# homenc/HElib

Hardware: NVIDIA H100
Metric: ctxt_mults_per_s (higher is better)
Workload: dtype u64

## Files before the change

### helib_b200/csrc/hb_device_v1.cuh

```cuda
#pragma once
#include <utility>
#include "hb_device.cuh"

#define HB1_RS 17
#define HB1_BS 273

__device__ __forceinline__ void hb_group_sync(int group, int nthreads) {
#ifdef HB_SIM
  cusim::bar_sync(1 + group, nthreads);
#else
  asm volatile("bar.sync %0, %1;" ::"r"(1 + group), "r"(nthreads) : "memory");
#endif
}

__device__ __forceinline__ void hb1_mac128(u64& hi, u64& lo, u64 a, u64 b) {
#ifdef HB_SIM
  hb_mac128(hi, lo, a, b);
#else
  asm("{\n\t.reg .u64 pl, ph;\n\t"
      "mul.lo.u64 pl, %2, %3;\n\t"
      "mul.hi.u64 ph, %2, %3;\n\t"
      "add.cc.u64 %0, %0, pl;\n\t"
      "addc.u64 %1, %1, ph;\n\t}"
      : "+l"(lo), "+l"(hi)
      : "l"(a), "l"(b));
#endif
}


__device__ __forceinline__ u64 hb1_mulwide(unsigned a, unsigned b) {
#ifdef HB_SIM
  return (u64)a * b;
#else
  u64 r; asm("mul.wide.u32 %0, %1, %2;" : "=l"(r) : "r"(a), "r"(b)); return r;
#endif
}
__device__ __forceinline__ u64 hb1_mulhi_approx(u64 a, u64 b) {
  const unsigned alo = (unsigned)a, ahi = (unsigned)(a >> 32), blo = (unsigned)b, bhi = (unsigned)(b >> 32);
  return hb1_mulwide(ahi, bhi) + (u64)__umulhi(alo, bhi) + (u64)__umulhi(ahi, blo);
}
struct Hb1Mod {
  u64 nq, qb, qb2;
  unsigned qt, qsh;
};
#define HB1_MOD(M, P) Hb1Mod M; M.nq = (P).nq; M.qb = (P).qb; M.qb2 = (P).qb + (P).qb; M.qt = (P).qt; M.qsh = (P).qsh
template <bool SP>
__device__ __forceinline__ u64 hb1_shoup4(u64 y, u64 w, u64 ws, const Hb1Mod& M) {
  const u64 hi = hb1_mulhi_approx(y, ws);
  if (SP) {
    const unsigned tl = (unsigned)hi * M.qt;
    const unsigned ylo = (unsigned)y, yhi = (unsigned)(y >> 32), wlo = (unsigned)w, whi = (unsigned)(w >> 32);
    const u64 R = hb1_mulwide(ylo, wlo) - hi;
    const unsigned rhi = (unsigned)(R >> 32) + yhi * wlo + ylo * whi - (tl << M.qsh);
    return ((u64)rhi << 32) | (unsigned)R;
  }
  return y * w + hi * M.nq;
}
__device__ __forceinline__ u64 hb1_csub(u64 x, u64 m) {
  const u64 d = x - m;
  return (i64)d < 0 ? x : d;
}
__device__ __forceinline__ u64 hb1_csub_hi(u64 x, u64 m) {
#ifdef HB_SIM
  if ((unsigned)(x >> 32) > (unsigned)(m >> 32)) x -= m;
  return x;
#else
  unsigned xl = (unsigned)x, xh = (unsigned)(x >> 32);
  asm("{ .reg .pred p; setp.gt.u32 p, %1, %3; @p sub.cc.u32 %0, %0, %2; @p subc.u32 %1, %1, %3; }"
      : "+r"(xl), "+r"(xh) : "r"((unsigned)m), "r"((unsigned)(m >> 32)));
  return ((u64)xh << 32) | xl;
#endif
}
template <bool SP>
__device__ __forceinline__ void hb1_ct(u64& x, u64& y, u64 w, u64 ws, const Hb1Mod& M) {
  const u64 xr = hb1_csub_hi(x, M.qb);
  const u64 t = hb1_shoup4<SP>(y, w, ws, M);
  x = xr + t;
  y = xr - t + M.qb;
}
template <bool SP>
__device__ __forceinline__ void hb1_gs(u64& x, u64& y, u64 w, u64 ws, const Hb1Mod& M) {
  const u64 s = x + y;
  const u64 d = x - y + M.qb2;
  x = hb1_csub_hi(s, M.qb);
  y = hb1_shoup4<SP>(d, w, ws, M);
}
__device__ __forceinline__ u64 hb1_canon4(u64 x, u64 q) {
  x = hb1_csub(x, q + q);
  return hb1_csub(x, q);
}
__device__ __forceinline__ u64 hb1_canon_fwd(u64 x, u64 q, u64 qb) {
  x = hb1_csub_hi(x, qb);
  x = hb1_csub(x, q + q);
  x = hb1_csub(x, q);
  return hb1_csub(x, q);
}
__device__ __forceinline__ u64 hb1_canon_inv(u64 x, u64 q) {
  x = hb1_csub(x, q + q);
  x = hb1_csub(x, q);
  return hb1_csub(x, q);
}

template <int I> struct HbC {
  static constexpr int value = I;
  __device__ constexpr operator int() const { return I; }
};
template <class F, int... I>
__device__ __forceinline__ void hb1_unroll_seq(F&& f, std::integer_sequence<int, I...>) { (f(HbC<I>{}), ...); }
template <int N, class F>
__device__ __forceinline__ void hb1_unroll(F&& f) { hb1_unroll_seq(f, std::make_integer_sequence<int, N>{}); }

struct Hb1TwReg {
  ulonglong2 t[15];
  template <int K, int G> __device__ __forceinline__ ulonglong2 get() const { return t[(1 << K) - 1 + G]; }
  template <class F> __device__ __forceinline__ void load(F&& f) {
    hb1_unroll<4>([&](auto k) { hb1_unroll<(1 << k)>([&](auto g) { t[(1 << k) - 1 + g] = f((int)k, (int)g); }); });
  }
};
struct Hb1TwPtr {
  const ulonglong2* p[4];
  template <int K, int G> __device__ __forceinline__ ulonglong2 get() const { return p[K][G]; }
};
template <bool SP, class TW>
__device__ __forceinline__ void hb1_r16_fwd(u64 (&a)[16], const TW& tw, const Hb1Mod& M) {
  hb1_unroll<4>([&](auto k) {
    constexpr int d = 8 >> k;
    hb1_unroll<(1 << k)>([&](auto g) {
      const ulonglong2 w = tw.template get<k, g>();
      hb1_unroll<d>([&](auto o) { hb1_ct<SP>(a[g * 2 * d + o], a[g * 2 * d + o + d], w.x, w.y, M); });
    });
  });
}
template <bool SP, class TW>
__device__ __forceinline__ void hb1_r16_inv(u64 (&a)[16], const TW& tw, const Hb1Mod& M) {
  hb1_unroll<4>([&](auto kr) {
    constexpr int k = 3 - kr, d = 8 >> k;
    hb1_unroll<(1 << k)>([&](auto g) {
      const ulonglong2 w = tw.template get<k, g>();
      hb1_unroll<d>([&](auto o) { hb1_gs<SP>(a[g * 2 * d + o], a[g * 2 * d + o + d], w.x, w.y, M); });
    });
  });
}
__device__ __forceinline__ unsigned hb1_brev4(unsigned x) {
  return ((x & 1u) << 3) | ((x & 2u) << 1) | ((x & 4u) >> 1) | ((x & 8u) >> 3);
}

struct Hb1BlkJob {
  int logN, epi, lazy;
  HbRows rows;
  u64 scal[HB_MAXROWS], scal_s[HB_MAXROWS];
  int nitems;
  const u64* src[HB_MAXB];
  u64* dst[HB_MAXB];
  u64* dst2[HB_MAXB];
};

__device__ __forceinline__ void hb1_cp8(u64* dst_smem, const u64* src) {
#ifdef HB_SIM
  *dst_smem = *src;
#else
  unsigned sa = (unsigned)__cvta_generic_to_shared(dst_smem);
  asm volatile("cp.async.ca.shared.global [%0], [%1], 8;" ::"r"(sa), "l"(src) : "memory");
#endif
}
__device__ __forceinline__ void hb1_cp_commit() {
#ifndef HB_SIM
  asm volatile("cp.async.commit_group;" ::: "memory");
#endif
}
template <int N> __device__ __forceinline__ void hb1_cp_wait() {
#ifndef HB_SIM
  asm volatile("cp.async.wait_group %0;" ::"n"(N) : "memory");
#endif
}

__device__ __forceinline__ void hb1_bulk_store128(u64* gdst, const u64* ssrc) {
#ifdef HB_SIM
  for (int i = 0; i < 16; i++) gdst[i] = ssrc[i];
#else
  asm volatile("cp.async.bulk.global.shared::cta.bulk_group [%0], [%1], 128;"
               ::"l"(gdst), "r"((unsigned)__cvta_generic_to_shared(ssrc)) : "memory");
  asm volatile("cp.async.bulk.commit_group;" ::: "memory");
#endif
}
__device__ __forceinline__ void hb1_fence_async() {
#ifndef HB_SIM
  asm volatile("fence.proxy.async.shared::cta;" ::: "memory");
#endif
}
__device__ __forceinline__ void hb1_bulk_wait_read() {
#ifndef HB_SIM
  asm volatile("cp.async.bulk.wait_group.read 0;" ::: "memory");
#endif
}
__device__ __forceinline__ void hb1_bulk_wait_all() {
#ifndef HB_SIM
  asm volatile("cp.async.bulk.wait_group 0;" ::: "memory");
#endif
}

#define HB1_STAGE (16 * HB1_BS + 8)

struct Hb1Unit { int rowi, ug, it; };
__device__ __forceinline__ Hb1Unit hb1_unit_next(Hb1Unit x, int G, int nitems) {
  if (++x.it == nitems) { x.it = 0; if (++x.ug == G) { x.ug = 0; ++x.rowi; } }
  return x;
}
__device__ __forceinline__ Hb1Unit hb1_unit(long u, int G, int nitems) {
  Hb1Unit x;
  const unsigned per_row = (unsigned)(G * nitems), uu = (unsigned)u;
  x.rowi = (int)(uu / per_row);
  const int rem = (int)(uu - (unsigned)x.rowi * per_row);
  x.ug = rem / nitems;
  x.it = rem - x.ug * nitems;
  return x;
}
__device__ __forceinline__ bool hb1_units(const Hb1BlkJob& J, int G, long& ubeg, long& uend) {
  const long U = (long)J.rows.n * G * J.nitems;
  ubeg = U * blockIdx.x / gridDim.x; uend = U * (blockIdx.x + 1) / gridDim.x;
  return ubeg < uend;
}
__device__ __forceinline__ Hb1TwPtr hb1_tw1(const ulonglong2* TW1, int tid) {
  Hb1TwPtr tw1;
  tw1.p[0] = TW1 + (tid >> 4) * 16; tw1.p[1] = tw1.p[0] + 1; tw1.p[2] = tw1.p[0] + 3; tw1.p[3] = tw1.p[0] + 7;
  return tw1;
}
__device__ __forceinline__ unsigned hb1_blk_reload(const HbPrimeDev& P, const ulonglong2* tw, int n1, int ug, int tid, Hb1Mod& M,
                                                   ulonglong2* TW1, Hb1TwReg& tw2) {
  const int blk1 = tid >> 4, lo = tid & 15, hi = tid >> 4, blk2 = tid & 15;
  M.nq = P.nq; M.qb = P.qb; M.qb2 = P.qb + P.qb; M.qt = P.qt; M.qsh = P.qsh;
  const unsigned b1 = hb_brev((ug << 4) + blk1, n1), b2 = hb_brev((ug << 4) + blk2, n1);
  if (lo < 15) {
    int e = lo, k = e >= 7 ? 3 : (e >= 3 ? 2 : (e >= 1 ? 1 : 0));
    int g = e - ((1 << k) - 1);
    TW1[blk1 * 16 + e] = tw[((size_t)1 << (n1 + k)) + ((size_t)b1 << k) + g];
  }
  tw2.load([&](int k, int g) { return tw[((size_t)1 << (n1 + 4 + k)) + ((size_t)b2 << (4 + k)) + ((size_t)hi << k) + g]; });
  __syncthreads();
  return b1;
}

template <bool SP>
__global__ void __launch_bounds__(256, 2) k1_fwd_blk(const HbPrimeDev* __restrict__ primes, const HB_GRID_CONSTANT Hb1BlkJob J) {
  HB_SMEM_DECL
  u64* S = HB_SMEM;
  u64* O = S + 2 * HB1_STAGE;
  ulonglong2* TW1 = (ulonglong2*)(O + 16 * 256);
  const int tid = threadIdx.x;
  const int n1 = J.logN - 8;
  const int G = 1 << (n1 - 4);
  long ubeg, uend;
  if (!hb1_units(J, G, ubeg, uend)) return;
  const int blk1 = tid >> 4, lo = tid & 15;
  const int hi = tid >> 4, blk2 = tid & 15;
  const unsigned hrev = hb1_brev4(hi);
  const bool epi1 = J.epi == 1, epi3 = J.epi == 3, lazy = J.lazy != 0;
  const int own = blk1 * HB1_BS + lo;
  const Hb1TwPtr tw1 = hb1_tw1(TW1, tid);

  auto src_ptr = [&](const Hb1Unit& x) {
    const unsigned b = hb_brev((x.ug << 4) + blk1, n1);
    return J.src[x.it] + ((size_t)J.rows.prime[x.rowi] << J.logN) + ((size_t)b << 8) + lo;
  };
  Hb1Unit cur = hb1_unit(ubeg, G, J.nitems);
  {
    const u64* src = src_ptr(cur);
    hb1_unroll<16>([&](auto r) { hb1_cp8(S + own + HB1_RS * r, src + 16 * r); });
  }
  hb1_cp_commit();
  int key = -1, buf = 0;
  u64 q = 0, sc = 0, sc_s = 0;
  Hb1Mod M; M.nq = 0; M.qb = 0; M.qb2 = 0; M.qt = 0; M.qsh = 0;
  Hb1TwReg tw2;
  for (long u = ubeg; u < uend; u++, buf ^= 1) {
    if (cur.rowi * G + cur.ug != key) {
      key = cur.rowi * G + cur.ug;
      const HbPrimeDev P = primes[J.rows.prime[cur.rowi]];
      q = P.q;
      sc = J.scal[cur.rowi]; sc_s = J.scal_s[cur.rowi];
      hb1_blk_reload(P, P.fw, n1, cur.ug, tid, M, TW1, tw2);
    }
    u64* Sb = S + buf * HB1_STAGE;
    const size_t doff = ((size_t)J.rows.prime[cur.rowi] << J.logN) + (cur.ug << 4) + blk2;
    u64* dst = J.dst[cur.it] + doff;
    const bool epi = epi1 || (epi3 && sc != 0);
    u64* old = epi3 ? J.dst2[cur.it] + doff : dst;
    if (epi) {
      hb1_unroll<16>([&](auto l) { hb1_cp8(O + l * 256 + tid, old + ((size_t)((hb1_brev4(l) << 4) | hrev) << n1)); });
    }
    hb1_cp_commit();
    Hb1Unit nxt = cur;
    if (u + 1 < uend) {
      nxt = hb1_unit_next(cur, G, J.nitems);
      const u64* src = src_ptr(nxt);
      u64* Sn = S + (buf ^ 1) * HB1_STAGE;
      hb1_unroll<16>([&](auto r) { hb1_cp8(Sn + own + HB1_RS * r, src + 16 * r); });
    }
    hb1_cp_commit();
    hb1_cp_wait<2>();
    u64 a[16];
    hb1_unroll<16>([&](auto r) { a[r] = Sb[own + HB1_RS * r]; });
    hb1_r16_fwd<SP>(a, tw1, M);
    hb1_unroll<16>([&](auto r) { Sb[own + HB1_RS * r] = a[r]; });
    __syncthreads();
    hb1_unroll<16>([&](auto l) { a[l] = Sb[blk2 * HB1_BS + HB1_RS * hi + l]; });
    hb1_r16_fwd<SP>(a, tw2, M);
    hb1_cp_wait<1>();
    hb1_unroll<16>([&](auto l) {
      if (epi) {
        u64 v = hb1_shoup4<SP>(O[l * 256 + tid] - a[l] + (M.qb2 + M.qb), sc, sc_s, M);
        if (!lazy) v = hb1_canon4(v, q);
        O[l * 256 + tid] = v;
      }
      if (!epi1 && !lazy) a[l] = hb1_canon_fwd(a[l], q, M.qb);
    });
    __syncthreads();
    if (!epi1) hb1_unroll<16>([&](auto l) { Sb[l * 256 + tid] = a[l]; });
    hb1_fence_async();
    __syncthreads();
    {
      const int l = tid >> 4, h = tid & 15;
      const size_t o = (size_t)((hb1_brev4(l) << 4) | hb1_brev4(h)) << n1;
      if (epi) hb1_bulk_store128(old - blk2 + o, O + l * 256 + 16 * h);
      if (!epi1) hb1_bulk_store128(dst - blk2 + o, Sb + l * 256 + 16 * h);
      hb1_bulk_wait_read();
    }
    __syncthreads();
    cur = nxt;
  }
  hb1_cp_wait<0>();
  hb1_bulk_wait_all();
}

template <bool SP, int NP>
__device__ __forceinline__ void hb1_fwd_blk_parts(const HbPrimeDev* __restrict__ primes, const Hb1BlkJob& J) {
  HB_SMEM_DECL
  u64* S = HB_SMEM;
  u64* O = S + 2 * HB1_STAGE;
  ulonglong2* TW1 = (ulonglong2*)(O + 16 * 256);
  u64* V = (u64*)(TW1 + 256);
  const int tid = threadIdx.x;
  const int n1 = J.logN - 8;
  const int G = 1 << (n1 - 4);
  long ubeg, uend;
  if (!hb1_units(J, G, ubeg, uend)) return;
  const int blk1 = tid >> 4, lo = tid & 15;
  const int hi = tid >> 4, blk2 = tid & 15;
  const unsigned hrev = hb1_brev4(hi);
  const int own = blk1 * HB1_BS + lo;
  u64* const Vt = V + tid;
  const Hb1TwPtr tw1 = hb1_tw1(TW1, tid);

  auto prefetch = [&](u64* Sn, const Hb1Unit& x, int k) {
    const unsigned b = hb_brev((x.ug << 4) + blk1, n1);
    const u64* src = J.src[NP * x.it + k] + ((size_t)J.rows.prime[x.rowi] << J.logN) + ((size_t)b << 8) + lo;
    hb1_unroll<16>([&](auto r) { hb1_cp8(Sn + own + HB1_RS * r, src + 16 * r); });
  };
  Hb1Unit cur = hb1_unit(ubeg, G, J.nitems);
  prefetch(S, cur, 0);
  hb1_cp_commit();
  int key = -1;
  u64 q = 0, sc = 0, sc_s = 0, c64 = 0, c64_s = 0, one_s = 0;
  Hb1Mod M; M.nq = 0; M.qb = 0; M.qb2 = 0; M.qt = 0; M.qsh = 0;
  Hb1TwReg tw2;
  for (long u = ubeg; u < uend; u++) {
    if (cur.rowi * G + cur.ug != key) {
      key = cur.rowi * G + cur.ug;
      const HbPrimeDev P = primes[J.rows.prime[cur.rowi]];
      q = P.q; c64 = P.c64; c64_s = P.c64_s; one_s = P.one_s;
      sc = J.scal[cur.rowi]; sc_s = J.scal_s[cur.rowi];
      hb1_blk_reload(P, P.fw, n1, cur.ug, tid, M, TW1, tw2);
    }
    const size_t doff = ((size_t)J.rows.prime[cur.rowi] << J.logN) + (cur.ug << 4) + blk2;
    u64* const* dst = J.dst + NP * cur.it;
    u64* const o2 = J.dst2[cur.it];
    const bool more = u + 1 < uend;
    const Hb1Unit nxt = more ? hb1_unit_next(cur, G, J.nitems) : cur;
#pragma unroll 1
    for (int k = 0; k < NP; k++) {
      u64* Sb = S + (NP == 2 ? k : k & 1) * HB1_STAGE;
      const u64* old = dst[k] + doff;
      hb1_unroll<16>([&](auto l) { hb1_cp8(O + l * 256 + tid, old + ((size_t)((hb1_brev4(l) << 4) | hrev) << n1)); });
      hb1_cp_commit();
      if (k < NP - 1) prefetch(S + ((k + 1) & 1) * HB1_STAGE, cur, k + 1);
      else if (more) prefetch(S, nxt, 0);
      hb1_cp_commit();
      hb1_cp_wait<2>();
      u64 a[16];
      hb1_unroll<16>([&](auto r) { a[r] = Sb[own + HB1_RS * r]; });
      hb1_r16_fwd<SP>(a, tw1, M);
      hb1_unroll<16>([&](auto r) { Sb[own + HB1_RS * r] = a[r]; });
      __syncthreads();
      hb1_unroll<16>([&](auto l) { a[l] = Sb[blk2 * HB1_BS + HB1_RS * hi + l]; });
      hb1_r16_fwd<SP>(a, tw2, M);
      hb1_cp_wait<1>();
      hb1_unroll<16>([&](auto l) {
        a[l] = hb1_shoup4<SP>(O[l * 256 + tid] - a[l] + (M.qb2 + M.qb), sc, sc_s, M);
      });
      if constexpr (NP == 4) {
        if (k < 2) {
          hb1_unroll<16>([&](auto l) { Vt[k * 4096 + l * 256] = a[l]; });
        } else if (k == 2) {
          hb1_unroll<16>([&](auto l) {
            const size_t o = doff + ((size_t)((hb1_brev4(l) << 4) | hrev) << n1);
            const u64 x0 = Vt[l * 256], x1 = Vt[4096 + l * 256], v = a[l];
            dst[0][o] = hb_reduce128(__umul64hi(x0, v), x0 * v, q, c64, c64_s, one_s);
            Vt[2 * 4096 + l * 256] = hb_reduce128(__umul64hi(x1, v), x1 * v, q, c64, c64_s, one_s);
          });
        } else {
          hb1_unroll<16>([&](auto l) {
            const size_t o = doff + ((size_t)((hb1_brev4(l) << 4) | hrev) << n1);
            const u64 x0 = Vt[l * 256], x1 = Vt[4096 + l * 256], v = a[l];
            u64 h = 0, w = Vt[2 * 4096 + l * 256];
            hb1_mac128(h, w, x0, v);
            dst[1][o] = hb_reduce128(h, w, q, c64, c64_s, one_s);
            dst[2][o] = hb_reduce128(__umul64hi(x1, v), x1 * v, q, c64, c64_s, one_s);
            dst[3][o] = v;
          });
        }
      } else {
        if (k == 0) {
          hb1_unroll<16>([&](auto l) { Vt[l * 256] = a[l]; });
        } else {
          hb1_unroll<16>([&](auto l) {
            const size_t o = doff + ((size_t)((hb1_brev4(l) << 4) | hrev) << n1);
            const u64 x0 = Vt[l * 256], v = a[l];
            u64 h = 0, w = 0;
            hb1_mac128(h, w, x0, v);
            hb1_mac128(h, w, x0, v);
            dst[0][o] = hb_reduce128(__umul64hi(x0, x0), x0 * x0, q, c64, c64_s, one_s);
            dst[1][o] = hb_reduce128(h, w, q, c64, c64_s, one_s);
            o2[o] = hb_reduce128(__umul64hi(v, v), v * v, q, c64, c64_s, one_s);
          });
        }
      }
      __syncthreads();
    }
    cur = nxt;
  }
  hb1_cp_wait<0>();
}
template <bool SP>
__global__ void __launch_bounds__(256, 1) k1_fwd_blk_tensor(const HbPrimeDev* __restrict__ primes, const HB_GRID_CONSTANT Hb1BlkJob J) {
  hb1_fwd_blk_parts<SP, 4>(primes, J);
}
template <bool SP>
__global__ void __launch_bounds__(256, 1) k1_fwd_blk_square(const HbPrimeDev* __restrict__ primes, const HB_GRID_CONSTANT Hb1BlkJob J) {
  hb1_fwd_blk_parts<SP, 2>(primes, J);
}

template <bool SP>
__global__ void __launch_bounds__(256, 2) k1_inv_blk(const HbPrimeDev* __restrict__ primes, const HB_GRID_CONSTANT Hb1BlkJob J) {
  HB_SMEM_DECL
  u64* S = HB_SMEM;
  ulonglong2* TW1 = (ulonglong2*)(S + 2 * HB1_STAGE);
  const int tid = threadIdx.x;
  const int n1 = J.logN - 8;
  const int G = 1 << (n1 - 4);
  long ubeg, uend;
  if (!hb1_units(J, G, ubeg, uend)) return;
  const int blk1 = tid >> 4, lo = tid & 15;
  const int hi = tid >> 4, blk2 = tid & 15;
  const unsigned hrev = hb1_brev4(hi);
  const Hb1TwPtr tw1 = hb1_tw1(TW1, tid);
  const int own = blk2 * HB1_BS + HB1_RS * hi;
  auto src_ptr = [&](const Hb1Unit& x) {
    return J.src[x.it] + ((size_t)J.rows.prime[x.rowi] << J.logN) + (x.ug << 4) + blk2;
  };
  Hb1Unit cur = hb1_unit(ubeg, G, J.nitems);
  {
    const u64* src = src_ptr(cur);
    hb1_unroll<16>([&](auto l) { hb1_cp8(S + own + l, src + ((size_t)((hb1_brev4(l) << 4) | hrev) << n1)); });
  }
  hb1_cp_commit();
  int key = -1, buf = 0;
  u64 q = 0;
  Hb1Mod M; M.nq = 0; M.qb = 0; M.qb2 = 0; M.qt = 0; M.qsh = 0;
  unsigned b1 = 0;
  Hb1TwReg tw2;
  for (long u = ubeg; u < uend; u++, buf ^= 1) {
    if (cur.rowi * G + cur.ug != key) {
      key = cur.rowi * G + cur.ug;
      const HbPrimeDev P = primes[J.rows.prime[cur.rowi]];
      q = P.q;
      b1 = hb1_blk_reload(P, P.iw, n1, cur.ug, tid, M, TW1, tw2);
    }
    u64* Sb = S + buf * HB1_STAGE;
    Hb1Unit nxt = cur;
    if (u + 1 < uend) {
      nxt = hb1_unit_next(cur, G, J.nitems);
      const u64* src = src_ptr(nxt);
      u64* Sn = S + (buf ^ 1) * HB1_STAGE;
      hb1_unroll<16>([&](auto l) { hb1_cp8(Sn + own + l, src + ((size_t)((hb1_brev4(l) << 4) | hrev) << n1)); });
    }
    hb1_cp_commit();
    hb1_cp_wait<1>();
    u64 a[16];
    hb1_unroll<16>([&](auto l) { a[l] = Sb[own + l]; });
    hb1_r16_inv<SP>(a, tw2, M);
    hb1_unroll<16>([&](auto l) { Sb[own + l] = a[l]; });
    __syncthreads();
    hb1_unroll<16>([&](auto r) { a[r] = Sb[blk1 * HB1_BS + HB1_RS * r + lo]; });
    hb1_r16_inv<SP>(a, tw1, M);
    u64* dst = J.dst[cur.it] + ((size_t)J.rows.prime[cur.rowi] << J.logN) + ((size_t)b1 << 8) + lo;
    hb1_unroll<16>([&](auto r) { dst[16 * r] = J.epi == 2 ? a[r] : hb1_canon_inv(a[r], q); });
    __syncthreads();
    cur = nxt;
  }
  hb1_cp_wait<0>();
}

struct Hb1ColsJob {
  int logN;
  HbRows rows;
  int nitems;
  const u64* src[HB_MAXB];
  u64* dst[HB_MAXB];
  int has_scal, npeers;
  u64 scal[HB_MAXROWS], scal_s[HB_MAXROWS];
  u64* peer[8][HB_MAXB];
};

template <bool SP>
__global__ void __launch_bounds__(256, 2) k1_fwd_cols(const HbPrimeDev* __restrict__ primes, const HB_GRID_CONSTANT Hb1ColsJob J) {
  HB_SMEM_DECL
  u64* T = HB_SMEM;
  const int tid = threadIdx.x;
  const int pi = J.rows.prime[blockIdx.y];
  const HbPrimeDev P = primes[pi];
  HB1_MOD(M, P);
  const size_t rowoff = (size_t)pi << J.logN;
  const unsigned c0 = blockIdx.x << 4;
  const int c = tid & 15, x = tid >> 4;
  Hb1TwPtr tw1;
  tw1.p[0] = P.fw + 1; tw1.p[1] = P.fw + 2; tw1.p[2] = P.fw + 4; tw1.p[3] = P.fw + 8;
  Hb1TwReg tw2;
  tw2.load([&](int k, int g) { return P.fw[(16 << k) + (x << k) + g]; });
  for (int it = blockIdx.z; it < J.nitems; it += gridDim.z) {
    const u64* src = J.src[it] + rowoff + c0 + c;
    u64* dst = J.dst[it] + rowoff + c0 + c;
    u64 a[16];
    hb1_unroll<16>([&](auto r) { a[r] = src[(size_t)(16 * r + x) << 8]; });
    hb1_r16_fwd<SP>(a, tw1, M);
    hb1_unroll<16>([&](auto r) { T[c * HB1_BS + HB1_RS * r + x] = a[r]; });
    __syncthreads();
    hb1_unroll<16>([&](auto l) { a[l] = T[c * HB1_BS + HB1_RS * x + l]; });
    hb1_r16_fwd<SP>(a, tw2, M);
    hb1_unroll<16>([&](auto l) { dst[(size_t)(16 * x + l) << 8] = a[l]; });
    __syncthreads();
  }
}
template <bool SP>
__global__ void __launch_bounds__(256, 2) k1_inv_cols(const HbPrimeDev* __restrict__ primes, const HB_GRID_CONSTANT Hb1ColsJob J) {
  HB_SMEM_DECL
  u64* T = HB_SMEM;
  const int tid = threadIdx.x;
  const int pi = J.rows.prime[blockIdx.y];
  const HbPrimeDev P = primes[pi];
  const u64 q = P.q; HB1_MOD(M, P);
  const size_t rowoff = (size_t)pi << J.logN;
  const unsigned c0 = blockIdx.x << 4;
  const int c = tid & 15, x = tid >> 4;
  Hb1TwPtr tw1;
  tw1.p[0] = P.iw + 1; tw1.p[1] = P.iw + 2; tw1.p[2] = P.iw + 4; tw1.p[3] = P.iw + 8;
  Hb1TwReg tw2;
  tw2.load([&](int k, int g) { return P.iw[(16 << k) + (x << k) + g]; });
  for (int it = blockIdx.z; it < J.nitems; it += gridDim.z) {
    const u64* src = J.src[it] + rowoff + c0 + c;
    u64* dst = J.dst[it] + rowoff + c0 + c;
    u64 a[16];
    hb1_unroll<16>([&](auto l) { a[l] = src[(size_t)(16 * x + l) << 8]; });
    hb1_r16_inv<SP>(a, tw2, M);
    hb1_unroll<16>([&](auto l) { T[c * HB1_BS + HB1_RS * x + l] = a[l]; });
    __syncthreads();
    hb1_unroll<16>([&](auto r) { a[r] = T[c * HB1_BS + HB1_RS * r + x]; });
    hb1_r16_inv<SP>(a, tw1, M);
    const u64 fm = J.has_scal ? J.scal[blockIdx.y] : P.ninv, fs = J.has_scal ? J.scal_s[blockIdx.y] : P.ninv_s;
    hb1_unroll<16>([&](auto r) {
      const u64 v = hb_mul_shoup(a[r], fm, fs, q);
      const size_t o = (size_t)(16 * r + x) << 8;
      dst[o] = v;
      for (int p = 0; p < J.npeers; p++) J.peer[p][it][rowoff + c0 + c + o] = v;
    });
    __syncthreads();
  }
}

#define HB1C_BS 276
#define HB1_TS (4 * HB1C_BS)
#define HB1_VS 260

struct Hb1ConvJob {
  const HbConvDev* cv;
  int logN, ngroups;
  int nitems;
  const u64* src[HB_MAXB];
  u64* dst[HB_MAXB];
  u64* stats;
  int src_is_y;
  double* frac[HB_MAXB];
};

template <bool SP>
__global__ void __launch_bounds__(640, 1) k1_conv(const HbPrimeDev* __restrict__ primes, const HB_GRID_CONSTANT Hb1ConvJob J) {
  HB_SMEM_DECL
  const HbConvDev* cv = J.cv;
  const int n = cv->n, nt = cv->nt, NG = J.ngroups;
  u64* Y = HB_SMEM;
  i64* Vb = (i64*)(Y + (size_t)n * HB1_TS);
  u64* W = (u64*)(Vb + 4 * HB1_VS);
  const int tid = threadIdx.x;
  const int grp = tid >> 6, gt = tid & 63;
  const int c = gt & 3, x = gt >> 2;
  const unsigned c0 = blockIdx.x << 2;
  const u64* src = J.src[blockIdx.y];
  u64* dst = J.dst[blockIdx.y];

  for (int j = grp; j < n; j += NG) {
    const int pi = cv->src_prime[j];
    const HbPrimeDev P = primes[pi];
    const u64 q = P.q; HB1_MOD(M, P);
    const u64* s = src + ((size_t)pi << J.logN) + c0 + c;
    u64* Yj = Y + (size_t)j * HB1_TS + c * HB1C_BS;
    u64 a[16];
    hb1_unroll<16>([&](auto l) { a[l] = s[(size_t)(16 * x + l) << 8]; });
    if (J.src_is_y) {
      hb1_unroll<16>([&](auto l) { Yj[HB1_RS * x + l] = a[l]; });
      continue;
    }
    {
      Hb1TwPtr tw;
      tw.p[0] = P.iw + 16 + x; tw.p[1] = P.iw + 32 + 2 * x; tw.p[2] = P.iw + 64 + 4 * x; tw.p[3] = P.iw + 128 + 8 * x;
      hb1_r16_inv<SP>(a, tw, M);
    }
    hb1_unroll<16>([&](auto l) { Yj[HB1_RS * x + l] = a[l]; });
    hb_group_sync(grp, 64);
    hb1_unroll<16>([&](auto r) { a[r] = Yj[HB1_RS * r + x]; });
    {
      Hb1TwPtr tw;
      tw.p[0] = P.iw + 1; tw.p[1] = P.iw + 2; tw.p[2] = P.iw + 4; tw.p[3] = P.iw + 8;
      hb1_r16_inv<SP>(a, tw, M);
    }
    const u64 t = cv->tn[j], ts = cv->tn_s[j];
    hb1_unroll<16>([&](auto r) { Yj[HB1_RS * r + x] = hb_mul_shoup(a[r], t, ts, q); });
  }
  __syncthreads();
  for (int e = tid; e < 1024; e += blockDim.x) {
    const int cc = e >> 8, i1 = e & 255;
    double* fr = J.frac[blockIdx.y];
    double f;
    Vb[cc * HB1_VS + i1] = hb_conv_v(cv, Y + cc * HB1C_BS + HB1_RS * (i1 >> 4) + (i1 & 15), HB1_TS, J.stats, fr ? &f : nullptr);
    if (fr) fr[((size_t)i1 << 8) + c0 + cc] = f;
  }
  __syncthreads();
  u64* Wg = W + (size_t)grp * HB1_TS + c * HB1C_BS;
  for (int t = grp; t < nt; t += NG) {
    const int pi = cv->tgt_prime[t];
    const HbPrimeDev P = primes[pi];
    HB1_MOD(M, P);
    const u64* ct = cv->c + (size_t)t * n;
    u64 a[16];
    {
      const u64 negq = cv->negQ[t], posq = cv->Qmod[t];
      hb1_unroll<2>([&](auto h) {
        u64 ahi[8], alo[8];
        hb1_unroll<8>([&](auto r) {
          const i64 v = Vb[c * HB1_VS + 16 * (8 * h + r) + x];
          const u64 m = v >= 0 ? (u64)v : (u64)(-v);
          const u64 f = v >= 0 ? negq : posq;
          if ((m >> 32) == 0) {
            const u64 p0 = hb1_mulwide((unsigned)m, (unsigned)f);
            const u64 p1 = hb1_mulwide((unsigned)m, (unsigned)(f >> 32)) + (p0 >> 32);
            alo[r] = (p1 << 32) | (unsigned)p0; ahi[r] = p1 >> 32;
          } else { alo[r] = m * f; ahi[r] = __umul64hi(m, f); }
        });
        for (int j = 0; j < n; j++) {
          const u64 cj = ct[j];
          const u64* Yj = Y + (size_t)j * HB1_TS + c * HB1C_BS + x + HB1_RS * 8 * h;
          hb1_unroll<8>([&](auto r) { hb1_mac128(ahi[r], alo[r], Yj[HB1_RS * r], cj); });
        }
        hb1_unroll<8>([&](auto r) { a[8 * h + r] = hb_reduce128_lazy(ahi[r], alo[r], P); });
      });
    }
    {
      Hb1TwPtr tw;
      tw.p[0] = P.fw + 1; tw.p[1] = P.fw + 2; tw.p[2] = P.fw + 4; tw.p[3] = P.fw + 8;
      hb1_r16_fwd<SP>(a, tw, M);
    }
    hb_group_sync(grp, 64);
    hb1_unroll<16>([&](auto r) { Wg[HB1_RS * r + x] = a[r]; });
    hb_group_sync(grp, 64);
    hb1_unroll<16>([&](auto l) { a[l] = Wg[HB1_RS * x + l]; });
    {
      Hb1TwPtr tw;
      tw.p[0] = P.fw + 16 + x; tw.p[1] = P.fw + 32 + 2 * x; tw.p[2] = P.fw + 64 + 4 * x; tw.p[3] = P.fw + 128 + 8 * x;
      hb1_r16_fwd<SP>(a, tw, M);
    }
    u64* d = dst + ((size_t)pi << J.logN) + c0 + c;
    hb1_unroll<16>([&](auto l) { d[(size_t)(16 * x + l) << 8] = a[l]; });
  }
}

struct Hb1Conv1Job {
  int logN, ngroups, cq, nitems;
  int src_prime, nt;
  int tgt_prime[HB_MAXROWS];
  u64 qs_mod[HB_MAXROWS];
  unsigned char nored[HB_MAXROWS];
  u64 ninv, ninv_s;
  const u64* src[HB_MAXB];
  u64* dst[HB_MAXB];
};
template <bool SP>
__global__ void __launch_bounds__(640, 1) k1_conv1(const HbPrimeDev* __restrict__ primes, const HB_GRID_CONSTANT Hb1Conv1Job J) {
  HB_SMEM_DECL
  const int NG = J.ngroups, CQ = J.cq, nt = J.nt;
  u64* Y = HB_SMEM;
  u64* W = Y + (size_t)CQ * HB1_TS;
  const int tid = threadIdx.x;
  const int grp = tid >> 6, gt = tid & 63;
  const int c = gt & 3, x = gt >> 2;
  const unsigned c0 = blockIdx.x * 4u * (unsigned)CQ;
  const u64* src = J.src[blockIdx.y];
  u64* dst = J.dst[blockIdx.y];
  const HbPrimeDev PS = primes[J.src_prime];
  for (int qd = grp; qd < CQ; qd += NG) {
    HB1_MOD(M, PS);
    const u64* s = src + ((size_t)J.src_prime << J.logN) + c0 + 4 * qd + c;
    u64* Yq = Y + (size_t)qd * HB1_TS + c * HB1C_BS;
    u64 a[16];
    hb1_unroll<16>([&](auto l) { a[l] = s[(size_t)(16 * x + l) << 8]; });
    {
      Hb1TwPtr tw;
      tw.p[0] = PS.iw + 16 + x; tw.p[1] = PS.iw + 32 + 2 * x; tw.p[2] = PS.iw + 64 + 4 * x; tw.p[3] = PS.iw + 128 + 8 * x;
      hb1_r16_inv<SP>(a, tw, M);
    }
    hb1_unroll<16>([&](auto l) { Yq[HB1_RS * x + l] = a[l]; });
    hb_group_sync(grp, 64);
    hb1_unroll<16>([&](auto r) { a[r] = Yq[HB1_RS * r + x]; });
    {
      Hb1TwPtr tw;
      tw.p[0] = PS.iw + 1; tw.p[1] = PS.iw + 2; tw.p[2] = PS.iw + 4; tw.p[3] = PS.iw + 8;
      hb1_r16_inv<SP>(a, tw, M);
    }
    hb1_unroll<16>([&](auto r) { Yq[HB1_RS * r + x] = hb_mul_shoup(a[r], J.ninv, J.ninv_s, PS.q); });
  }
  __syncthreads();
  const u64 qs_half = (PS.q - 1) >> 1;
  u64* Wg = W + (size_t)grp * HB1_TS + c * HB1C_BS;
  for (int w = grp; w < nt * CQ; w += NG) {
    const int t = w / CQ, qd = w - t * CQ;
    const int pi = J.tgt_prime[t];
    const HbPrimeDev P = primes[pi];
    HB1_MOD(M, P);
    const u64 adj = P.q - J.qs_mod[t];
    const u64* Yq = Y + (size_t)qd * HB1_TS + c * HB1C_BS + x;
    const bool nored = J.nored[t] != 0;
    u64 a[16];
    hb1_unroll<16>([&](auto r) {
      const u64 y = Yq[HB1_RS * r];
      u64 v = nored ? y : y - __umul64hi(y, P.one_s) * P.q;
      if (y > qs_half) v += adj;
      a[r] = v;
    });
    {
      Hb1TwPtr tw;
      tw.p[0] = P.fw + 1; tw.p[1] = P.fw + 2; tw.p[2] = P.fw + 4; tw.p[3] = P.fw + 8;
      hb1_r16_fwd<SP>(a, tw, M);
    }
    hb_group_sync(grp, 64);
    hb1_unroll<16>([&](auto r) { Wg[HB1_RS * r + x] = a[r]; });
    hb_group_sync(grp, 64);
    hb1_unroll<16>([&](auto l) { a[l] = Wg[HB1_RS * x + l]; });
    {
      Hb1TwPtr tw;
      tw.p[0] = P.fw + 16 + x; tw.p[1] = P.fw + 32 + 2 * x; tw.p[2] = P.fw + 64 + 4 * x; tw.p[3] = P.fw + 128 + 8 * x;
      hb1_r16_fwd<SP>(a, tw, M);
    }
    u64* d = dst + ((size_t)pi << J.logN) + c0 + 4 * qd + c;
    hb1_unroll<16>([&](auto l) { d[(size_t)(16 * x + l) << 8] = a[l]; });
  }
}

__device__ __forceinline__ ulonglong2 hb1_ld2(const u64* p) { return *reinterpret_cast<const ulonglong2*>(p); }
__device__ __forceinline__ void hb1_st2(u64* p, u64 x, u64 y) { ulonglong2 v; v.x = x; v.y = y; *reinterpret_cast<ulonglong2*>(p) = v; }
template <int ND>
__global__ void __launch_bounds__(256) k1_ks_inner(const HbPrimeDev* __restrict__ primes, const HB_GRID_CONSTANT HbKsJob J) {
  const int pi = J.rows.prime[blockIdx.y];
  const HbPrimeDev P = primes[pi];
  const size_t o = (size_t)pi * (size_t)J.N + 2 * ((size_t)blockIdx.x * 256 + threadIdx.x);
  ulonglong2 ea[ND], eb[ND];
#pragma unroll
  for (int i = 0; i < ND; i++) { ea[i] = hb1_ld2(J.evk_a[i] + o); eb[i] = hb1_ld2(J.evk_b[i] + o); }
  const int own = J.own_dig[blockIdx.y];
  const u64 sc = J.scal[blockIdx.y];
  const bool rd = J.mode == 0 || sc != 0;
  for (int it = blockIdx.z; it < J.nitems; it += gridDim.z) {
    ulonglong2 d[ND];
#pragma unroll
    for (int i = 0; i < ND; i++) d[i] = hb1_ld2((i == own ? J.own[it] : J.dig[it][i]) + o);
    u64 h0x = 0, l0x = 0, h0y = 0, l0y = 0, h1x = 0, l1x = 0, h1y = 0, l1y = 0;
    if (rd) {
      const ulonglong2 p0 = hb1_ld2(J.out0[it] + o), p1 = hb1_ld2(J.out1[it] + o);
      if (J.mode == 0) { l0x = p0.x; l0y = p0.y; l1x = p1.x; l1y = p1.y; }
      else { hb1_mac128(h0x, l0x, p0.x, sc); hb1_mac128(h0y, l0y, p0.y, sc); hb1_mac128(h1x, l1x, p1.x, sc); hb1_mac128(h1y, l1y, p1.y, sc); }
    }
#pragma unroll
    for (int i = 0; i < ND; i++) {
      hb1_mac128(h0x, l0x, d[i].x, eb[i].x); hb1_mac128(h0y, l0y, d[i].y, eb[i].y);
      hb1_mac128(h1x, l1x, d[i].x, ea[i].x); hb1_mac128(h1y, l1y, d[i].y, ea[i].y);
    }
    hb1_st2(J.out0[it] + o, hb_reduce128(h0x, l0x, P), hb_reduce128(h0y, l0y, P));
    hb1_st2(J.out1[it] + o, hb_reduce128(h1x, l1x, P), hb_reduce128(h1y, l1y, P));
  }
}

struct Hb1TensorJob {
  u64 N;
  HbRows rows;
  int nitems;
  const u64* a0[HB_MAXB]; const u64* a1[HB_MAXB]; const u64* b0[HB_MAXB]; const u64* b1[HB_MAXB];
  u64* o0[HB_MAXB]; u64* o1[HB_MAXB]; u64* o2[HB_MAXB];
};
__global__ void __launch_bounds__(256) k1_tensor(const HbPrimeDev* __restrict__ primes, const HB_GRID_CONSTANT Hb1TensorJob J) {
  const int pi = J.rows.prime[blockIdx.y];
  const HbPrimeDev P = primes[pi];
  const int it = blockIdx.z;
  const size_t o = (size_t)pi * (size_t)J.N + 2 * ((size_t)blockIdx.x * 256 + threadIdx.x);
  const ulonglong2 a0 = hb1_ld2(J.a0[it] + o), a1 = hb1_ld2(J.a1[it] + o), b0 = hb1_ld2(J.b0[it] + o), b1 = hb1_ld2(J.b1[it] + o);
  u64 hx = 0, lx = 0, hy = 0, ly = 0;
  hb1_mac128(hx, lx, a0.x, b1.x); hb1_mac128(hx, lx, a1.x, b0.x);
  hb1_mac128(hy, ly, a0.y, b1.y); hb1_mac128(hy, ly, a1.y, b0.y);
  hb1_st2(J.o0[it] + o, hb_mulmod(a0.x, b0.x, P), hb_mulmod(a0.y, b0.y, P));
  hb1_st2(J.o1[it] + o, hb_reduce128(hx, lx, P), hb_reduce128(hy, ly, P));
  hb1_st2(J.o2[it] + o, hb_mulmod(a1.x, b1.x, P), hb_mulmod(a1.y, b1.y, P));
}

#define HB_TSUM_GROUP 127
#define HB_TSUM_SLOTS 128
struct Hb1TensorSumJob {
  u64 N;
  HbRows rows;
  int npairs, nitems, accumulate;
  const u64* a0[HB_TSUM_SLOTS]; const u64* a1[HB_TSUM_SLOTS]; const u64* b0[HB_TSUM_SLOTS]; const u64* b1[HB_TSUM_SLOTS];
  u64* o0[HB_MAXB]; u64* o1[HB_MAXB]; u64* o2[HB_MAXB];
};
__device__ __forceinline__ u64 hb1_canon(u64 x, const HbPrimeDev& P) {
  u64 r = x - __umul64hi(x, P.one_s) * P.q;
  return r >= P.q ? r - P.q : r;
}
__global__ void __launch_bounds__(256) k1_tensor_sum(const HbPrimeDev* __restrict__ primes, const HB_GRID_CONSTANT Hb1TensorSumJob J) {
  const int pi = J.rows.prime[blockIdx.y];
  const HbPrimeDev P = primes[pi];
  const int it = blockIdx.z;
  const size_t o = (size_t)pi * (size_t)J.N + 2 * ((size_t)blockIdx.x * 256 + threadIdx.x);
  u64 h0x = 0, l0x = 0, h0y = 0, l0y = 0, h1x = 0, l1x = 0, h1y = 0, l1y = 0, h2x = 0, l2x = 0, h2y = 0, l2y = 0;
  if (J.accumulate) {
    const ulonglong2 p0 = hb1_ld2(J.o0[it] + o), p1 = hb1_ld2(J.o1[it] + o), p2 = hb1_ld2(J.o2[it] + o);
    l0x = p0.x; l0y = p0.y; l1x = p1.x; l1y = p1.y; l2x = p2.x; l2y = p2.y;
  }
  const int s0 = it * J.npairs;
  for (int j0 = 0; j0 < J.npairs; j0 += HB_TSUM_GROUP) {
    if (j0 > 0) {
      l0x = hb_reduce128(h0x, l0x, P); l0y = hb_reduce128(h0y, l0y, P); l1x = hb_reduce128(h1x, l1x, P);
      l1y = hb_reduce128(h1y, l1y, P); l2x = hb_reduce128(h2x, l2x, P); l2y = hb_reduce128(h2y, l2y, P);
      h0x = h0y = h1x = h1y = h2x = h2y = 0;
    }
    const int j1 = J.npairs - j0 < HB_TSUM_GROUP ? J.npairs : j0 + HB_TSUM_GROUP;
    for (int j = j0; j < j1; j++) {
      const int s = s0 + j;
      const ulonglong2 A0 = hb1_ld2(J.a0[s] + o), A1 = hb1_ld2(J.a1[s] + o), B0 = hb1_ld2(J.b0[s] + o), B1 = hb1_ld2(J.b1[s] + o);
      const u64 a0x = hb1_canon(A0.x, P), a0y = hb1_canon(A0.y, P), a1x = hb1_canon(A1.x, P), a1y = hb1_canon(A1.y, P);
      const u64 b0x = hb1_canon(B0.x, P), b0y = hb1_canon(B0.y, P), b1x = hb1_canon(B1.x, P), b1y = hb1_canon(B1.y, P);
      hb1_mac128(h0x, l0x, a0x, b0x); hb1_mac128(h0y, l0y, a0y, b0y);
      hb1_mac128(h1x, l1x, a0x, b1x); hb1_mac128(h1x, l1x, a1x, b0x);
      hb1_mac128(h1y, l1y, a0y, b1y); hb1_mac128(h1y, l1y, a1y, b0y);
      hb1_mac128(h2x, l2x, a1x, b1x); hb1_mac128(h2y, l2y, a1y, b1y);
    }
  }
  hb1_st2(J.o0[it] + o, hb_reduce128(h0x, l0x, P), hb_reduce128(h0y, l0y, P));
  hb1_st2(J.o1[it] + o, hb_reduce128(h1x, l1x, P), hb_reduce128(h1y, l1y, P));
  hb1_st2(J.o2[it] + o, hb_reduce128(h2x, l2x, P), hb_reduce128(h2y, l2y, P));
}
```

Measured before the change: 3061.

## Use 30-bit limb split with 32-bit wide multiplies in conv inner product

```diff
diff --git a/bench_micro/ubench_conv.cu b/bench_micro/ubench_conv.cu
--- /dev/null
+++ b/bench_micro/ubench_conv.cu
@@ -0,0 +1,92 @@
+#define HB_CONV_MARKS
+#include <cstdio>
+#include <cstdlib>
+#include <algorithm>
+#include <cstring>
+#include <vector>
+#include "hb_device_v1.cuh"
+
+#define CK(x) do { cudaError_t e_ = (x); if (e_ != cudaSuccess) { printf("%s:%d %s\n", __FILE__, __LINE__, cudaGetErrorString(e_)); exit(1); } } while (0)
+
+static u64 rng_state = 0x9E3779B97F4A7C15ull;
+static u64 rnd() { rng_state ^= rng_state << 13; rng_state ^= rng_state >> 7; rng_state ^= rng_state << 17; return rng_state; }
+static u64 shoup(u64 w, u64 q) { return (u64)(((unsigned __int128)w << 64) / q); }
+template <class T> static T* up(const std::vector<T>& v) { T* d; CK(cudaMalloc(&d, v.size() * sizeof(T))); CK(cudaMemcpy(d, v.data(), v.size() * sizeof(T), cudaMemcpyHostToDevice)); return d; }
+
+int main() {
+  const int logN = 16, N = 1 << logN, NPR = 30, NG = 10;
+  int nsm = 0; CK(cudaDeviceGetAttribute(&nsm, cudaDevAttrMultiProcessorCount, 0));
+  std::vector<HbPrimeDev> P(NPR);
+  std::vector<u64> qs(NPR);
+  for (int i = 0; i < NPR; i++) {
+    const u64 qt = (1u << 19) + 2 * i + 1, q = (qt << 40) + 1;
+    qs[i] = q;
+    std::vector<ulonglong2> fw(N), iw(N);
+    for (int k = 0; k < N; k++) { u64 a = rnd() % q, b = rnd() % q; fw[k] = make_ulonglong2(a, shoup(a, q)); iw[k] = make_ulonglong2(b, shoup(b, q)); }
+    HbPrimeDev& p = P[i];
+    p.q = q; p.ninv = rnd() % q; p.ninv_s = shoup(p.ninv, q);
+    p.c64 = (u64)(((unsigned __int128)1 << 64) % q); p.c64_s = shoup(p.c64, q); p.one_s = (u64)(~0ull / q);
+    p.nq = 0 - q; p.qb = 4 * q; p.qt = (unsigned)qt; p.qsh = 8;
+    p.fw = up(fw); p.iw = up(iw);
+  }
+  HbPrimeDev* dP = up(P);
+  const int shapes[3][3] = {{10, 19, 32}, {9, 20, 32}, {10, 19, 64}};
+  const char* names[3] = {"digit 1: 10 -> 19 x 32", "digit 2:  9 -> 20 x 32", "mod-down: 10 -> 19 x 64"};
+  const int maxit = 64;
+  u64 *src, *dst, *stats;
+  const size_t per = (size_t)NPR * N;
+  CK(cudaMalloc(&src, per * maxit * 8)); CK(cudaMalloc(&dst, per * maxit * 8)); CK(cudaMalloc(&stats, 8));
+  {
+    std::vector<u64> h(per);
+    for (int it = 0; it < maxit; it++) {
+      for (size_t k = 0; k < per; k++) h[k] = rnd() % qs[k / N];
+      CK(cudaMemcpy(src + per * it, h.data(), per * 8, cudaMemcpyHostToDevice));
+    }
+  }
+  CK(cudaFuncSetAttribute(k1_conv<true>, cudaFuncAttributeMaxDynamicSharedMemorySize, 227 * 1024));
+  cudaEvent_t e0, e1; CK(cudaEventCreate(&e0)); CK(cudaEventCreate(&e1));
+  printf("k1_conv, N = 2^16, %d SMs, %d groups of 64 threads; best of 5 launches\n", nsm, NG);
+  double tot = 0;
+  for (int s = 0; s < 3; s++) {
+    const int n = shapes[s][0], nt = shapes[s][1], nit = shapes[s][2];
+    std::vector<int> sp(n), tp(nt);
+    std::vector<u64> tn(n), tns(n), fm(n), c((size_t)nt * n), nq(nt), qm(nt), zero(8, 0);
+    std::vector<int> fsh(n);
+    for (int j = 0; j < n; j++) { sp[j] = j; tn[j] = rnd() % qs[j]; tns[j] = shoup(tn[j], qs[j]); fm[j] = (u64)(((unsigned __int128)1 << 123) / qs[j]); fsh[j] = 59; }
+    for (int t = 0; t < nt; t++) {
+      tp[t] = n + t; nq[t] = rnd() % qs[n + t]; qm[t] = qs[n + t] - nq[t];
+      for (int j = 0; j < n; j++) c[(size_t)t * n + j] = rnd() % qs[n + t];
+    }
+    HbConvDev H; memset(&H, 0, sizeof(H));
+    H.n = n; H.nt = nt; H.L = 8; H.src_prime = up(sp); H.tgt_prime = up(tp); H.tn = up(tn); H.tn_s = up(tns); H.fmul = up(fm);
+    H.fshift = up(fsh); H.c = up(c); H.negQ = up(nq); H.Qmod = up(qm); H.Q = up(zero); H.Qhalf = up(zero); H.Qj = up(std::vector<u64>((size_t)n * 8, 0));
+    HbConvDev* dH = up(std::vector<HbConvDev>(1, H));
+    Hb1ConvJob J; memset(&J, 0, sizeof(J));
+    J.cv = dH; J.logN = logN; J.ngroups = NG; J.nitems = nit; J.stats = stats;
+    for (int i = 0; i < nit; i++) { J.src[i] = src + per * i; J.dst[i] = dst + per * i; }
+    const size_t smem = ((size_t)(n + NG) * HB1_TS + 4 * HB1_VS) * 8;
+    float best = 1e30f;
+    for (int r = 0; r < 6; r++) {
+      CK(cudaEventRecord(e0));
+      k1_conv<true><<<dim3(64, nit), 64 * NG, smem>>>(dP, J);
+      CK(cudaEventRecord(e1)); CK(cudaEventSynchronize(e1)); CK(cudaGetLastError());
+      float ms; CK(cudaEventElapsedTime(&ms, e0, e1));
+      if (r > 0 && ms < best) best = ms;
+    }
+    tot += best;
+    printf("%-26s grid %4d x %2d  smem %6zu B  %.3f ms\n", names[s], 64, nit, smem, best);
+    static const unsigned long long z[128] = {};
+    CK(cudaMemcpyToSymbol(hb_conv_marks, z, sizeof(z)));
+    k1_conv<true><<<dim3(64, nit), 64 * NG, smem>>>(dP, J);
+    CK(cudaDeviceSynchronize());
+    unsigned long long m[128];
+    CK(cudaMemcpyFromSymbol(m, hb_conv_marks, sizeof(m)));
+    double ph[4] = {0, 0, 0, 0}, nu = 0;
+    for (int g = 0; g < NG; g++) { for (int k = 0; k < 4; k++) ph[k] += (double)m[g * 8 + k]; nu += (double)m[g * 8 + 4]; }
+    const double sum = ph[0] + ph[1] + ph[2] + ph[3];
+    printf("  cycles per CTA (mean over groups):  sources %.0f (%.1f%%)  quotient %.0f (%.1f%%)  own targets %.0f (%.1f%%)  end wait %.0f (%.1f%%)\n",
+           ph[0] / nu, 100 * ph[0] / sum, ph[1] / nu, 100 * ph[1] / sum, ph[2] / nu, 100 * ph[2] / sum, ph[3] / nu, 100 * ph[3] / sum);
+  }
+  printf("step total %.3f ms\n", tot);
+  return 0;
+}
diff --git a/helib_b200/csrc/hb_device_v1.cuh b/helib_b200/csrc/hb_device_v1.cuh
--- a/helib_b200/csrc/hb_device_v1.cuh
+++ b/helib_b200/csrc/hb_device_v1.cuh
@@ -24,6 +24,15 @@
       "addc.u64 %1, %1, ph;\n\t}"
       : "+l"(lo), "+l"(hi)
       : "l"(a), "l"(b));
+#endif
+}
+
+__device__ __forceinline__ void hb1_add128(u64& hi, u64& lo, u64 bhi, u64 blo) {
+#ifdef HB_SIM
+  lo += blo;
+  hi += bhi + (lo < blo ? 1ull : 0ull);
+#else
+  asm("add.cc.u64 %0, %0, %2;\n\taddc.u64 %1, %1, %3;" : "+l"(lo), "+l"(hi) : "l"(blo), "l"(bhi));
 #endif
 }
 
@@ -601,6 +610,15 @@
   double* frac[HB_MAXB];
 };
 
+#ifdef HB_CONV_MARKS
+__device__ unsigned long long hb_conv_marks[16 * 8];
+#define HB_CONV_MARK(t) const long long t = clock64()
+#define HB_CONV_ADD(k, v) do { if (gt == 0) atomicAdd(&hb_conv_marks[grp * 8 + (k)], (unsigned long long)(v)); } while (0)
+#else
+#define HB_CONV_MARK(t)
+#define HB_CONV_ADD(k, v) do {} while (0)
+#endif
+
 template <bool SP>
 __global__ void __launch_bounds__(640, 1) k1_conv(const HbPrimeDev* __restrict__ primes, const HB_GRID_CONSTANT Hb1ConvJob J) {
   HB_SMEM_DECL
@@ -615,6 +633,7 @@
   const unsigned c0 = blockIdx.x << 2;
   const u64* src = J.src[blockIdx.y];
   u64* dst = J.dst[blockIdx.y];
+  HB_CONV_MARK(tm0);
 
   for (int j = grp; j < n; j += NG) {
     const int pi = cv->src_prime[j];
@@ -645,6 +664,7 @@
     hb1_unroll<16>([&](auto r) { Yj[HB1_RS * r + x] = hb_mul_shoup(a[r], t, ts, q); });
   }
   __syncthreads();
+  HB_CONV_MARK(tm1);
   for (int e = tid; e < 1024; e += blockDim.x) {
     const int cc = e >> 8, i1 = e & 255;
     double* fr = J.frac[blockIdx.y];
@@ -653,6 +673,7 @@
     if (fr) fr[((size_t)i1 << 8) + c0 + cc] = f;
   }
   __syncthreads();
+  HB_CONV_MARK(tm2);
   u64* Wg = W + (size_t)grp * HB1_TS + c * HB1C_BS;
   for (int t = grp; t < nt; t += NG) {
     const int pi = cv->tgt_prime[t];
@@ -662,25 +683,54 @@
     u64 a[16];
     {
       const u64 negq = cv->negQ[t], posq = cv->Qmod[t];
-      hb1_unroll<2>([&](auto h) {
-        u64 ahi[8], alo[8];
-        hb1_unroll<8>([&](auto r) {
-          const i64 v = Vb[c * HB1_VS + 16 * (8 * h + r) + x];
-          const u64 m = v >= 0 ? (u64)v : (u64)(-v);
-          const u64 f = v >= 0 ? negq : posq;
-          if ((m >> 32) == 0) {
-            const u64 p0 = hb1_mulwide((unsigned)m, (unsigned)f);
-            const u64 p1 = hb1_mulwide((unsigned)m, (unsigned)(f >> 32)) + (p0 >> 32);
-            alo[r] = (p1 << 32) | (unsigned)p0; ahi[r] = p1 >> 32;
-          } else { alo[r] = m * f; ahi[r] = __umul64hi(m, f); }
+      auto v_term = [&](int i, u64& hi, u64& lo) {
+        const i64 v = Vb[c * HB1_VS + 16 * i + x];
+        const u64 m = v >= 0 ? (u64)v : (u64)(-v);
+        const u64 f = v >= 0 ? negq : posq;
+        if ((m >> 32) == 0) {
+          const u64 p0 = hb1_mulwide((unsigned)m, (unsigned)f);
+          const u64 p1 = hb1_mulwide((unsigned)m, (unsigned)(f >> 32)) + (p0 >> 32);
+          lo = (p1 << 32) | (unsigned)p0; hi = p1 >> 32;
+        } else { lo = m * f; hi = __umul64hi(m, f); }
+      };
+      if (n <= 16) {
+        hb_group_sync(grp, 64);
+        hb1_unroll<4>([&](auto h) {
+          u64 s0[4], s1[4], s2[4], s3[4];
+          hb1_unroll<4>([&](auto r) { s0[r] = 0; s1[r] = 0; s2[r] = 0; s3[r] = 0; });
+          for (int j = 0; j < n; j++) {
+            const u64 cj = ct[j];
+            const unsigned cl = (unsigned)cj & 0x3fffffffu, ch = (unsigned)(cj >> 30);
+            const u64* Yj = Y + (size_t)j * HB1_TS + c * HB1C_BS + x + HB1_RS * 4 * h;
+            hb1_unroll<4>([&](auto r) {
+              const u64 y = Yj[HB1_RS * r];
+              const unsigned yl = (unsigned)y & 0x3fffffffu, yh = (unsigned)(y >> 30);
+              s0[r] += hb1_mulwide(yl, cl); s1[r] += hb1_mulwide(yl, ch); s2[r] += hb1_mulwide(yh, cl); s3[r] += hb1_mulwide(yh, ch);
+            });
+          }
+          hb1_unroll<4>([&](auto r) {
+            u64 hi, lo;
+            v_term(4 * h + r, hi, lo);
+            const u64 mid = s1[r] + s2[r], mc = mid < s1[r] ? 1ull : 0ull;
+            hb1_add128(hi, lo, (mc << 30) | (mid >> 34), mid << 30);
+            hb1_add128(hi, lo, s3[r] >> 4, s3[r] << 60);
+            hb1_add128(hi, lo, 0, s0[r]);
+            Wg[HB1_RS * (4 * h + r) + x] = hb_reduce128_lazy(hi, lo, P);
+          });
         });
-        for (int j = 0; j < n; j++) {
-          const u64 cj = ct[j];
-          const u64* Yj = Y + (size_t)j * HB1_TS + c * HB1C_BS + x + HB1_RS * 8 * h;
-          hb1_unroll<8>([&](auto r) { hb1_mac128(ahi[r], alo[r], Yj[HB1_RS * r], cj); });
-        }
-        hb1_unroll<8>([&](auto r) { a[8 * h + r] = hb_reduce128_lazy(ahi[r], alo[r], P); });
-      });
+        hb1_unroll<16>([&](auto r) { a[r] = Wg[HB1_RS * r + x]; });
+      } else {
+        hb1_unroll<2>([&](auto h) {
+          u64 ahi[8], alo[8];
+          hb1_unroll<8>([&](auto r) { v_term(8 * h + r, ahi[r], alo[r]); });
+          for (int j = 0; j < n; j++) {
+            const u64 cj = ct[j];
+            const u64* Yj = Y + (size_t)j * HB1_TS + c * HB1C_BS + x + HB1_RS * 8 * h;
+            hb1_unroll<8>([&](auto r) { hb1_mac128(ahi[r], alo[r], Yj[HB1_RS * r], cj); });
+          }
+          hb1_unroll<8>([&](auto r) { a[8 * h + r] = hb_reduce128_lazy(ahi[r], alo[r], P); });
+        });
+      }
     }
     {
       Hb1TwPtr tw;
@@ -699,6 +749,12 @@
     u64* d = dst + ((size_t)pi << J.logN) + c0 + c;
     hb1_unroll<16>([&](auto l) { d[(size_t)(16 * x + l) << 8] = a[l]; });
   }
+#ifdef HB_CONV_MARKS
+  HB_CONV_MARK(tm3);
+  __syncthreads();
+  HB_CONV_MARK(tm4);
+  HB_CONV_ADD(0, tm1 - tm0); HB_CONV_ADD(1, tm2 - tm1); HB_CONV_ADD(2, tm3 - tm2); HB_CONV_ADD(3, tm4 - tm3); HB_CONV_ADD(4, 1);
+#endif
 }
 
 struct Hb1Conv1Job {
```

Result: no change. 3072 (median of 6 runs) (+0.4%).
